# cyyever/distributed_learning_simulation_lib

Measured on AMD Instinct MI355X. Metric: aggregated GB/s (device-resident), N-client weighted FedAvg reduce, 1/2/4/8 GPU, higher is better.
Workload: dtype f64; 1 GPU; fedavg_resnet18_fp32_64_clients; clients_per_gpu=64, total_clients=64, clients_per_launch=64, client_table=prepared once (persistent client slots), params_per_client=11689512, tensors_per_client=62, in_dtype=float32, accumulate_dtype=float64, out_dtype=float32, parallelism=single GPU

## Files before the change

### distributed_learning_simulation_lib_amd/build.py

```python

from __future__ import annotations

import os
import shutil
import subprocess
from pathlib import Path

PKG_DIR = Path(__file__).resolve().parent
REPO_DIR = PKG_DIR.parent
CSRC = PKG_DIR / "csrc"
LIB_DIR = PKG_DIR / "_lib"
LIB_NAME = "libfedavg_hip.so"
LIB_PATH = LIB_DIR / LIB_NAME
SOURCES = [CSRC / "fedavg_kernels.hip", CSRC / "personalized_kernels.hip", CSRC / "robust_kernels.hip",
           CSRC / "krum_kernels.hip", CSRC / "point_kernels.hip", CSRC / "clip_kernels.hip", CSRC / "host_pack.cpp",
           CSRC / "sharded_comm.cpp", CSRC / "multi_device.cpp"]
HEADERS = [REPO_DIR / "include" / "fedavg_hip.h", CSRC / "exact_div.h", CSRC / "rccl_bind.h",
           CSRC / "robust_internal.h", CSRC / "krum_internal.h", CSRC / "point_internal.h", CSRC / "clip_internal.h"]
EXAMPLES = {"c_abi_round": REPO_DIR / "examples" / "c_abi_round.cpp",
            "multi_device_round": REPO_DIR / "examples" / "multi_device_round.cpp",
            "threaded_ranks": REPO_DIR / "tests" / "native" / "threaded_ranks.cpp"}
FAKE_RCCL_SRC = REPO_DIR / "tests" / "native" / "fake_rccl.cpp"
FAKE_RCCL = {"libfake_rccl.so": [], "libfake_rccl_nogather.so": ["-DFAKE_RCCL_NO_GATHER"]}
STAGING_SRC = CSRC / "staging_ext.cpp"
STAGING_NAME = "fedavg_staging"
STAGING_DIR = LIB_DIR / "staging"
STAGING_PATH = STAGING_DIR / f"{STAGING_NAME}.so"

HIPCC_FLAGS = [
    "--offload-arch=gfx950",
    "-O3",
    "-std=c++17",
    "-ffp-contract=off",
    "-fPIC",
    "-shared",
    "-Wall",
    "-Wno-unused-function",
]


def hipcc() -> str:
    cand = os.environ.get("HIPCC") or shutil.which("hipcc") or "/opt/rocm/bin/hipcc"
    return cand


def needs_build() -> bool:
    if not LIB_PATH.exists():
        return True
    mtime = LIB_PATH.stat().st_mtime
    return any(p.stat().st_mtime > mtime for p in SOURCES + HEADERS + [Path(__file__)])

# ... 74 lines not shown
```

### distributed_learning_simulation_lib_amd/csrc/fedavg_kernels.hip

```cpp
#include <hip/hip_runtime.h>
#include <hip/hip_ext.h>
#include <hip/hip_fp16.h>

#include <algorithm>
#include <atomic>
#include <chrono>
#include <cmath>
#include <cstdint>
#include <cstdio>
#include <cstdlib>
#include <cstring>
#include <limits>
#include <mutex>
#include <string>
#include <type_traits>
#include <vector>

#include "../../include/fedavg_hip.h"
#include "exact_div.h"
#include "robust_internal.h"
#include "krum_internal.h"
#include "point_internal.h"
#include "clip_internal.h"

namespace {

thread_local std::string g_last_error;

int32_t fail(int32_t code, const std::string& msg) {
  g_last_error = msg;
  return code;
}

#define FEDAVG_HIP_TRY(expr)                                                              \
  do {                                                                                    \
    hipError_t e_ = (expr);                                                               \
    if (e_ != hipSuccess) {                                                               \
      return fail(FEDAVG_ERR_HIP, std::string(#expr) + ": " + hipGetErrorString(e_));     \
    }                                                                                     \
  } while (0)

constexpr int kThreads = 256;
#ifndef FEDAVG_AE
#define FEDAVG_AE 16
#endif
#ifndef FEDAVG_AE_HALF
#define FEDAVG_AE_HALF 16
#endif
#ifndef FEDAVG_AE_F64
#define FEDAVG_AE_F64 8
#endif
#ifndef FEDAVG_TILE1
#define FEDAVG_TILE1 4096
#endif
#ifndef FEDAVG_CU_BYTES
#define FEDAVG_CU_BYTES 256
#endif
#ifndef FEDAVG_CU_BYTES_F64
#define FEDAVG_CU_BYTES_F64 512
#endif
#ifndef FEDAVG_PIPE
#define FEDAVG_PIPE 1
#endif
#ifndef FEDAVG_ACC_PLAIN_STORE_HALF
#define FEDAVG_ACC_PLAIN_STORE_HALF 1
#endif
#ifndef FEDAVG_BALANCE_DEFAULT
#define FEDAVG_BALANCE_DEFAULT 3
#endif
#ifndef FEDAVG_WALK_ALTERNATE
#define FEDAVG_WALK_ALTERNATE 1
#endif
#ifndef FEDAVG_PIPE_BYTES
#define FEDAVG_PIPE_BYTES 64
#endif
constexpr int kAE = FEDAVG_AE;
constexpr int kTile1 = FEDAVG_TILE1;
#ifndef FEDAVG_TILE_WIDE
#define FEDAVG_TILE_WIDE 8192
#endif
constexpr int kTileWide = FEDAVG_TILE_WIDE;
constexpr int kTile4 = (kThreads / 4) * kAE;

struct TileDesc {
  int32_t seg;
  int32_t count;
  int64_t start;
};

struct SegDesc {
  int64_t acc_off;
  int64_t numel;
};

struct CallTables {
  const void* const* cptrs;
  const double* w;
  const int32_t* kseg;
  const int32_t* acc_in;
  void* const* outs;
  const double* wtot;
  const void* const* base;
};

struct KArgs {
  const TileDesc* tiles;
  const SegDesc* segs;
  CallTables tab;
  double* acc;
  uint32_t* flag;
  int32_t tile_begin;
  int32_t num_tiles;
  int32_t K;
  int32_t zero_init;
  int32_t walk_back;
  const double* qtab;
  int32_t qtab_seg0;
  double* const* win_dst;
  const int32_t* win_edge;
  int32_t win_n;
  const double* const* comb_src;
// ... 108 lines not shown
  return (kptr<T>)(p);
}

__device__ __forceinline__ TileDesc load_tile(const TileDesc* tiles, int64_t i) {
  const kptr<int32_t> p = to_const<int32_t>(tiles + i);
  TileDesc d;
  d.seg = p[0];
  d.count = p[1];
  d.start = to_const<int64_t>(tiles + i)[1];
  return d;
}

template <typename T>
__device__ __forceinline__ double load_g(gptr<const T> p, int64_t i);
template <>
__device__ __forceinline__ double load_g<float>(gptr<const float> p, int64_t i) { return p[i]; }
template <>
__device__ __forceinline__ double load_g<double>(gptr<const double> p, int64_t i) { return p[i]; }
template <>
__device__ __forceinline__ double load_g<__half>(gptr<const __half> p, int64_t i) {
  return half_bits_to_f64(((gptr<const uint16_t>)p)[i]);
}
template <>
__device__ __forceinline__ double load_g<bf16_t>(gptr<const bf16_t> p, int64_t i) {
  return bf16_bits_to_f64(((gptr<const uint16_t>)p)[i]);
}

template <typename T, int LANES, bool FULL, bool VEC, int AE>
struct LaneLoader {
  using V = typename Vec16<T>::type;
  static constexpr int N = Vec16<T>::n;
  static constexpr int VPL = AE / N;

  __device__ __forceinline__ static void load_raw(gptr<const T> base, int li, V (&buf)[VPL], int nv = VPL) {
    const gptr<const V> vb = (gptr<const V>)base;
#pragma unroll
    for (int v = 0; v < VPL; ++v) {
      if (FULL || v < nv) {
        buf[v] = __builtin_nontemporal_load(vb + v * LANES + li);
      } else {
        buf[v] = V{};
      }
    }
  }

  __device__ __forceinline__ static void load_checked(gptr<const T> base, int li, int count,
                                                      double (&x)[AE]) {
#pragma unroll
    for (int v = 0; v < VPL; ++v) {
      const int e = (v * LANES + li) * N;
      if (VEC && e + N <= count) {
        const V raw = ((gptr<const V>)base)[v * LANES + li];
        expand<T>(raw, x + v * N);
      } else {
#pragma unroll
        for (int j = 0; j < N; ++j) x[v * N + j] = (e + j < count) ? load_g<T>(base, e + j) : 0.0;
      }
    }
  }
};

template <typename T, int SPLIT, int TILEN = kTile1>
struct Geo {
  static constexpr int AE = (SPLIT > 1) ? kAE
                          : (sizeof(T) == 2 ? FEDAVG_AE_HALF
                             : sizeof(T) == 8 ? FEDAVG_AE_F64
                                              : kAE);
  static constexpr int LANES = (SPLIT > 1) ? 64 : TILEN / AE;
  static constexpr int THREADS = (SPLIT > 1) ? kThreads : LANES;
  static constexpr int TILE = LANES * AE;
  static_assert(SPLIT == 1 || TILE == kTile4, "split tiles");
  static_assert(SPLIT > 1 || TILE == TILEN, "tile geometry");
  static_assert(THREADS % 64 == 0 && THREADS <= 1024, "workgroup size");
};

__device__ __forceinline__ void raise_flag(uint32_t* flag, int word) {
  __hip_atomic_store(flag + word, 1u, __ATOMIC_RELAXED, __HIP_MEMORY_SCOPE_SYSTEM);
}

template <typename V>
__device__ __forceinline__ void store_out(gptr<V> p, V v) {
  __builtin_nontemporal_store(v, p);
}

enum FoldKind : int { FOLD_MULADD = 0, FOLD_FMA = 1, FOLD_DELTA = 2 };

template <int FOLD>
__device__ __forceinline__ double fold(double acc, double x, double w, double base) {
  if constexpr (FOLD == FOLD_FMA) {
    return __builtin_fma(x, w, acc);
  } else if constexpr (FOLD == FOLD_DELTA) {
    const double full = base + x;
    const double p = full * w;
    return acc + p;
  } else {
    const double p = x * w;
    return acc + p;
  }
}

template <typename T, int OUT, int SPLIT, bool VEC, bool FULL, int FOLD, int TILEN = kTile1, bool PARTV = false,
          bool COMB = false>
__device__ __forceinline__ void tile_body(const KArgs& a, const TileDesc& td, double* lds) {
  constexpr int AE = Geo<T, SPLIT, TILEN>::AE;
  constexpr int LANES = Geo<T, SPLIT, TILEN>::LANES;
  using LL = LaneLoader<T, LANES, FULL && VEC, VEC, AE>;
  using V = typename LL::V;
  constexpr int N = LL::N;
  constexpr int VPL = LL::VPL;
  constexpr int CU_B = sizeof(T) == 8 ? FEDAVG_CU_BYTES_F64 : FEDAVG_CU_BYTES;
  constexpr int CU_LOADS = (CU_B / (VPL * 16)) < 2 ? 2 : (CU_B / (VPL * 16));
  constexpr bool FAST = (FULL || PARTV) && VEC;

  const int seg = td.seg;
  const int count = td.count;
  const int nv = FULL ? VPL : count / (LANES * N);
  const int wave = __builtin_amdgcn_readfirstlane(static_cast<int>(threadIdx.x) >> 6);
  const int li = (SPLIT == 1) ? static_cast<int>(threadIdx.x) : static_cast<int>(threadIdx.x & 63);

  const int kseg = to_const<int32_t>(a.tab.kseg)[seg];
  int kb = 0, ke = kseg;
  if constexpr (SPLIT > 1) {
    const int per = (kseg + SPLIT - 1) / SPLIT;
    kb = min(kseg, wave * per);
    ke = min(kseg, kb + per);
  }
  const kptr<uint64_t> cp = to_const<uint64_t>(a.tab.cptrs) + static_cast<int64_t>(seg) * a.K;
  const kptr<double> wp = to_const<double>(a.tab.w) + static_cast<int64_t>(seg) * a.K;
  const int64_t acc_base = to_const<int64_t>(a.segs)[2 * seg] + td.start;
  const int64_t elem_off = td.start * static_cast<int64_t>(sizeof(T));
  auto client = [&](int k) -> gptr<const T> {
    return to_global<T>(reinterpret_cast<const void*>(cp[k] + elem_off));
  };

  double acc[AE];
#pragma unroll
  for (int i = 0; i < AE; ++i) acc[i] = -0.0;
  bool have = a.zero_init != 0;
  if ((SPLIT == 1 || wave == 0) && !a.zero_init && to_const<int32_t>(a.tab.acc_in)[seg]) {
    const gptr<const double> ap = to_global<double>(a.acc + acc_base);
#pragma unroll
    for (int v = 0; v < VPL; ++v) {
      const int e = (v * LANES + li) * N;
#pragma unroll
      for (int j = 0; j < N; j += 2) {
        if (FULL || e + j + 2 <= count) {
          const f64x2 d = *(gptr<const f64x2>)(ap + e + j);
          acc[v * N + j] = d.x;
          acc[v * N + j + 1] = d.y;
        } else {
          if (e + j < count) acc[v * N + j] = ap[e + j];
          if (e + j + 1 < count) acc[v * N + j + 1] = ap[e + j + 1];
        }
      }
    }
    have = true;
  }

  double base[AE];
#pragma unroll
  for (int i = 0; i < AE; ++i) base[i] = 0.0;
  if constexpr (FOLD == FOLD_DELTA) {
    const gptr<const double> bp =
        to_global<double>(reinterpret_cast<const void*>(to_const<uint64_t>(a.tab.base)[seg])) + td.start;
#pragma unroll
    for (int v = 0; v < VPL; ++v) {
      const int e = (v * LANES + li) * N;
#pragma unroll
      for (int j = 0; j < N; j += 2) {
        if (VEC && (FULL || e + j + 2 <= count)) {
          const f64x2 d = *(gptr<const f64x2>)(bp + e + j);
          base[v * N + j] = d.x;
          base[v * N + j + 1] = d.y;
        } else {
          if (e + j < count) base[v * N + j] = bp[e + j];
          if (e + j + 1 < count) base[v * N + j + 1] = bp[e + j + 1];
        }
      }
    }
  }

  constexpr bool PIPE = FAST && ((FEDAVG_PIPE >> (sizeof(T) == 2 ? 0 : sizeof(T) == 4 ? 1 : 2)) & 1);
  if constexpr (PIPE) {
    constexpr int PB = FEDAVG_PIPE_BYTES;
    constexpr int PG = (PB / (VPL * 16)) < 1 ? 1 : (PB / (VPL * 16));
    V bufA[PG][VPL], bufB[PG][VPL];
    double wA[PG], wB[PG];
    auto load_stage = [&](V (&buf)[PG][VPL], double (&wk)[PG], int k) {
#pragma unroll
      for (int c = 0; c < PG; ++c) {
        const int kc = min(k + c, ke - 1);
        wk[c] = wp[kc];
        LL::load_raw(client(kc), li, buf[c], nv);
      }
    };
    auto fold_stage = [&](auto tail_tag, V (&buf)[PG][VPL], const double (&wk)[PG], int n) {
      constexpr bool TAIL = decltype(tail_tag)::value;
#pragma unroll
      for (int c = 0; c < PG; ++c) {
#pragma unroll
        for (int v = 0; v < VPL; ++v) {
          double x[N];
          expand<T>(buf[c][v], x);
#pragma unroll
          for (int j = 0; j < N; ++j) {
            double& r = acc[v * N + j];
            const double nv = fold<FOLD>(r, x[j], wk[c], base[v * N + j]);
            if constexpr (TAIL) {
              r = (c < n) ? nv : r;
            } else {
              r = nv;
            }
          }
        }
      }
    };
    if (kb < ke) {
      int k = kb;
      load_stage(bufA, wA, k);
      while (k + 2 * PG <= ke) {
        load_stage(bufB, wB, k + PG);
        fold_stage(std::false_type{}, bufA, wA, PG);
        load_stage(bufA, wA, k + 2 * PG);
        fold_stage(std::false_type{}, bufB, wB, PG);
        k += 2 * PG;
      }
      if (k + PG < ke) {
        load_stage(bufB, wB, k + PG);
        fold_stage(std::false_type{}, bufA, wA, PG);
        fold_stage(std::true_type{}, bufB, wB, ke - k - PG);
      } else if (k < ke) {
        fold_stage(std::true_type{}, bufA, wA, ke - k);
      }
    }
  } else if constexpr (FAST) {
    auto group = [&](auto tail_tag, int k, int n) {
      constexpr bool TAIL = decltype(tail_tag)::value;
      V buf[CU_LOADS][VPL];
      double wk[CU_LOADS];
#pragma unroll
      for (int c = 0; c < CU_LOADS; ++c) {
        const int kc = TAIL ? k + min(c, n - 1) : k + c;
        wk[c] = wp[kc];
        LL::load_raw(client(kc), li, buf[c], nv);
      }
#pragma unroll
      for (int c = 0; c < CU_LOADS; ++c) {
#pragma unroll
        for (int v = 0; v < VPL; ++v) {
          double x[N];
          expand<T>(buf[c][v], x);
#pragma unroll
          for (int j = 0; j < N; ++j) {
            double& r = acc[v * N + j];
            const double nv = fold<FOLD>(r, x[j], wk[c], base[v * N + j]);
            if constexpr (TAIL) {
              r = (c < n) ? nv : r;
            } else {
              r = nv;
            }
          }
        }
      }
    };
    int k = kb;
    for (; k + CU_LOADS <= ke; k += CU_LOADS) group(std::false_type{}, k, CU_LOADS);
    if (k < ke) group(std::true_type{}, k, ke - k);
  } else {
    for (int k = kb; k < ke; ++k) {
      const double wk = wp[k];
      double x[AE];
      LL::load_checked(client(k), li, count, x);
#pragma unroll
      for (int i = 0; i < AE; ++i) acc[i] = fold<FOLD>(acc[i], x[i], wk, base[i]);
    }
  }
  have = have || (ke > kb);

  if constexpr (SPLIT > 1) {
    int* have_lds = reinterpret_cast<int*>(lds + (SPLIT - 1) * 64 * AE);
    if (wave > 0) {
      double* dst = lds + ((wave - 1) * 64 + li) * AE;
#pragma unroll
      for (int i = 0; i < AE; ++i) dst[i] = acc[i];
      if (li == 0) have_lds[wave - 1] = have ? 1 : 0;
    }
    __syncthreads();
    if (wave != 0) return;
#pragma unroll
    for (int w2 = 1; w2 < SPLIT; ++w2) {
      if (have_lds[w2 - 1]) {
        const double* src = lds + ((w2 - 1) * 64 + li) * AE;
        if (have) {
#pragma unroll
          for (int i = 0; i < AE; ++i) acc[i] = acc[i] + src[i];
        } else {
#pragma unroll
          for (int i = 0; i < AE; ++i) acc[i] = src[i];
        }
        have = true;
      }
    }
  }
  if (!have) return;

  if constexpr (COMB) {
    static_assert(OUT != OUT_ACC && SPLIT == 1, "the own-window combine ends a final fold");
    double tot[AE];
#pragma unroll
    for (int i = 0; i < AE; ++i) tot[i] = -0.0;
    for (int h = 0; h < a.comb_n; ++h) {
      if (h == a.comb_self) {
#pragma unroll
        for (int i = 0; i < AE; ++i) tot[i] = tot[i] + acc[i];
      } else {
        const gptr<const double> sp =
            to_global<double>(reinterpret_cast<const void*>(to_const<uint64_t>(a.comb_src)[h])) + acc_base;
#pragma unroll
        for (int v = 0; v < VPL; ++v) {
          const int e = (v * LANES + li) * N;
#pragma unroll
          for (int j = 0; j < N; j += 2) {
            if (FULL || e + j + 2 <= count) {
              const f64x2 d = *(gptr<const f64x2>)(sp + e + j);
              tot[v * N + j] = tot[v * N + j] + d.x;
              tot[v * N + j + 1] = tot[v * N + j + 1] + d.y;
            } else {
              if (e + j < count) tot[v * N + j] = tot[v * N + j] + sp[e + j];
              if (e + j + 1 < count) tot[v * N + j + 1] = tot[v * N + j + 1] + sp[e + j + 1];
            }
          }
        }
      }
    }
#pragma unroll
    for (int i = 0; i < AE; ++i) acc[i] = tot[i];
  }

  bool bad_acc = false;
#pragma unroll
  for (int v = 0; v < VPL; ++v) {
    const int e = (v * LANES + li) * N;
#pragma unroll
    for (int j = 0; j < N; ++j) {
      const bool in_range = FULL || (e + j < count);
      bad_acc |= in_range && (acc[v * N + j] != acc[v * N + j]);
    }
  }

  if constexpr (OUT == OUT_ACC) {
    const gptr<double> ap = to_global_mut<double>(a.acc + acc_base);
#pragma unroll
    for (int v = 0; v < VPL; ++v) {
      const int e = (v * LANES + li) * N;
#pragma unroll
      for (int j = 0; j < N; j += 2) {
        if (FULL || e + j + 2 <= count) {
          const f64x2 pair = f64x2{acc[v * N + j], acc[v * N + j + 1]};
          if constexpr (sizeof(T) == 2 && FEDAVG_ACC_PLAIN_STORE_HALF) {
            *(gptr<f64x2>)(ap + e + j) = pair;
          } else {
            store_out((gptr<f64x2>)(ap + e + j), pair);
          }
        } else {
          if (e + j < count) ap[e + j] = acc[v * N + j];
          if (e + j + 1 < count) ap[e + j + 1] = acc[v * N + j + 1];
        }
      }
    }
    if (__ballot(bad_acc) != 0ull && (threadIdx.x & 63) == 0) raise_flag(a.flag, 0);
  } else {
    const double W = to_const<double>(a.tab.wtot)[seg];
    bool bad_res = false;
    double res[AE];
    exact_div_block<AE>(acc, res, W);
#pragma unroll
    for (int v = 0; v < VPL; ++v) {
      const int e = (v * LANES + li) * N;
#pragma unroll
      for (int j = 0; j < N; ++j) {
        const bool in_range = FULL || (e + j < count);
        bad_res |= in_range && (res[v * N + j] != res[v * N + j]);
      }
    }
    void* const out_raw = reinterpret_cast<void*>(to_const<uint64_t>(a.tab.outs)[seg]);
    if constexpr (OUT == OUT_F32) {
      const gptr<float> op = to_global_mut<float>(out_raw) + td.start;
#pragma unroll
      for (int v = 0; v < VPL; ++v) {
        const int e = (v * LANES + li) * N;
        if constexpr (N >= 4) {
#pragma unroll
          for (int j = 0; j < N; j += 4) {
            if (VEC && (FULL || e + j + 4 <= count)) {
              store_out((gptr<f32x4>)(op + e + j),
                  f32x4{static_cast<float>(res[v * N + j]), static_cast<float>(res[v * N + j + 1]),
                        static_cast<float>(res[v * N + j + 2]), static_cast<float>(res[v * N + j + 3])});
            } else {
#pragma unroll
              for (int q = 0; q < 4; ++q)
                if (e + j + q < count) op[e + j + q] = static_cast<float>(res[v * N + j + q]);
            }
          }
        } else {
          if (VEC && (FULL || e + 2 <= count)) {
            store_out((gptr<f32x2>)(op + e),
                      f32x2{static_cast<float>(res[v * N]), static_cast<float>(res[v * N + 1])});
          } else {
            if (e < count) op[e] = static_cast<float>(res[v * N]);
            if (e + 1 < count) op[e + 1] = static_cast<float>(res[v * N + 1]);
          }
        }
      }
    } else {
      const gptr<double> op = to_global_mut<double>(out_raw) + td.start;
#pragma unroll
      for (int v = 0; v < VPL; ++v) {
        const int e = (v * LANES + li) * N;
#pragma unroll
        for (int j = 0; j < N; j += 2) {
          if (VEC && (FULL || e + j + 2 <= count)) {
            store_out((gptr<f64x2>)(op + e + j), f64x2{res[v * N + j], res[v * N + j + 1]});
          } else {
            if (e + j < count) op[e + j] = res[v * N + j];
            if (e + j + 1 < count) op[e + j + 1] = res[v * N + j + 1];
          }
        }
      }
    }
    const uint64_t ba = __ballot(bad_acc);
    const uint64_t br = __ballot(bad_res);
    if ((ba | br) != 0ull && (threadIdx.x & 63) == 0) {
      if (ba) raise_flag(a.flag, 0);
      if (br) raise_flag(a.flag, 1);
    }
  }
}

template <typename T, int OUT, int SPLIT, bool VEC, int FOLD, int TILEN = kTile1, bool PV = false, bool COMB = false>
__global__ __launch_bounds__((Geo<T, SPLIT, TILEN>::THREADS)) void fedavg_tile_kernel(KArgs a) {
  __shared__ double lds[(SPLIT > 1) ? ((SPLIT - 1) * 64 * kAE + 8) : 1];
  constexpr int TILE = Geo<T, SPLIT, TILEN>::TILE;
  const int ntiles = (SPLIT == 1) ? a.num_tiles : static_cast<int>(gridDim.x);
  if constexpr (OUT == OUT_ACC && SPLIT == 1) {
    if (a.win_dst != nullptr) {
      for (int t = blockIdx.x; t < ntiles; t += gridDim.x) {
        const int32_t ti = a.tile_begin + t;
        const kptr<int32_t> we = to_const<int32_t>(a.win_edge);
        int j = 0;
        while (j + 1 < a.win_n && ti >= we[j + 1]) ++j;
        KArgs b = a;
        b.acc = reinterpret_cast<double*>(to_const<uint64_t>(a.win_dst)[j]);
        const TileDesc td = load_tile(a.tiles, ti);
        if (td.count == TILE) tile_body<T, OUT, SPLIT, VEC, true, FOLD, TILEN>(b, td, lds);
        else tile_body<T, OUT, SPLIT, VEC, false, FOLD, TILEN>(b, td, lds);
      }
      return;
    }
  }
  if constexpr (COMB) {
    const TileDesc td = load_tile(a.tiles, a.tile_begin + static_cast<int>(blockIdx.x));
    if (td.count == TILE) tile_body<T, OUT, SPLIT, VEC, true, FOLD, TILEN, false, true>(a, td, lds);
    else tile_body<T, OUT, SPLIT, VEC, false, FOLD, TILEN, false, true>(a, td, lds);
    return;
  }
  for (int t = blockIdx.x; t < ntiles; t += gridDim.x) {
    const TileDesc td = load_tile(a.tiles, a.tile_begin + (t < a.walk_back ? a.walk_back - 1 - t : t));
    constexpr int LV = Geo<T, SPLIT, TILEN>::LANES * Vec16<T>::n;
    if (td.count == TILE) {
      tile_body<T, OUT, SPLIT, VEC, true, FOLD, TILEN>(a, td, lds);
    } else {
      bool partv = false;
      if constexpr (PV && SPLIT == 1 && VEC && LV < TILE) partv = (td.count % LV) == 0;
      if (partv) {
        if constexpr (PV && SPLIT == 1 && VEC && LV < TILE) tile_body<T, OUT, SPLIT, VEC, false, FOLD, TILEN, true>(a, td, lds);
      } else {
        tile_body<T, OUT, SPLIT, VEC, false, FOLD, TILEN>(a, td, lds);
      }
    }
    if constexpr (SPLIT > 1) break;
  }
}

struct DynCtl {
  uint64_t word;
  uint64_t pad[7];
};
struct DynAck {
  uint64_t word;
  uint32_t error;
  uint32_t polls;
  uint64_t t_seen;
  uint64_t t_done;
  uint64_t t_rows;
};
struct DynMirror {
  uint64_t word;
  uint64_t pad[7];
};
constexpr int kDynCopies = 8;
constexpr int kDynMirrorSleep = 8;
constexpr int kDynTileSleep = 32;
__host__ __device__ constexpr uint64_t dyn_word(uint32_t count, uint32_t closed, uint32_t mode, uint32_t epoch) {
  return static_cast<uint64_t>(count & 0xffffffu) | (static_cast<uint64_t>(closed & 1u) << 24) |
         (static_cast<uint64_t>(mode & 7u) << 25) | (static_cast<uint64_t>(epoch) << 32);
}
struct DynArgs {
  const TileDesc* tiles;
  const TileDesc* edge_tiles;
  const SegDesc* segs;
  double* acc;
// ... 1155 lines not shown

namespace {

constexpr size_t align_up(size_t x, size_t a) { return (x + a - 1) / a * a; }

struct DynLayout {
  size_t ctl, ack, wtot, outs, wtab, ptab, bytes;
  DynLayout(int T, int cap) {
    ctl = 0;
    ack = align_up(ctl + sizeof(DynCtl), 64);
    wtot = align_up(ack + sizeof(DynAck), 64);
    outs = align_up(wtot + sizeof(double) * T, 64);
    wtab = align_up(outs + sizeof(uint64_t) * T, 64);
    ptab = align_up(wtab + sizeof(double) * cap, 64);
    bytes = align_up(ptab + sizeof(uint64_t) * static_cast<size_t>(T) * cap, 4096);
  }
};


int32_t elem_size(int32_t dt) {
  switch (dt) {
    case FEDAVG_F32: return 4;
    case FEDAVG_F16: return 2;
    case FEDAVG_BF16: return 2;
    case FEDAVG_F64: return 8;
    case FEDAVG_QSGD_F32: return 1;
    case FEDAVG_QSGD_F64: return 1;
    case FEDAVG_NNADQ_F32: return 1;
    case FEDAVG_NNADQ_F64: return 1;
    default: return 0;
  }
}

int32_t build_balanced_tiles(const std::vector<int64_t>& numel, int tile, int gran, int64_t slots,
                             std::vector<TileDesc>& out) {
  std::vector<TileDesc> full, tail;
  int64_t tail_elems = 0;
  for (size_t t = 0; t < numel.size(); ++t) {
    const int64_t q = numel[t] / tile;
    for (int64_t i = 0; i < q; ++i) full.push_back(TileDesc{static_cast<int32_t>(t), tile, i * tile});
    int64_t start = q * tile, r = numel[t] - q * tile;
    const int64_t rv = r - r % gran;
    if (rv > 0) {
      tail.push_back(TileDesc{static_cast<int32_t>(t), static_cast<int32_t>(rv), start});
      start += rv;
      r -= rv;
      tail_elems += rv;
    }
    if (r > 0) {
      tail.push_back(TileDesc{static_cast<int32_t>(t), static_cast<int32_t>(r), start});
      tail_elems += r;
    }
  }
  slots = std::max<int64_t>(slots, 1);
  const int64_t head = (static_cast<int64_t>(full.size()) / slots) * slots;
  const int64_t rest = static_cast<int64_t>(full.size()) - head;
  const int64_t remaining = rest * tile + tail_elems;
  int64_t piece = (remaining + slots - 1) / slots;
  piece = std::min<int64_t>(tile, std::max<int64_t>(gran, (piece + gran - 1) / gran * gran));
  out.assign(full.begin(), full.begin() + head);
  std::vector<TileDesc> end;
  for (int64_t i = head; i < static_cast<int64_t>(full.size()); ++i) {
    for (int64_t s = 0; s < tile; s += piece) {
      const int64_t c = std::min<int64_t>(piece, tile - s);
      end.push_back(TileDesc{full[i].seg, static_cast<int32_t>(c), full[i].start + s});
    }
  }
  end.insert(end.end(), tail.begin(), tail.end());
  std::stable_sort(end.begin(), end.end(), [](const TileDesc& a, const TileDesc& b) { return a.count > b.count; });
  out.insert(out.end(), end.begin(), end.end());
  return static_cast<int32_t>(head);
}

void build_tiles(const std::vector<int64_t>& numel, int tile, std::vector<TileDesc>& out) {
  out.clear();
  for (size_t t = 0; t < numel.size(); ++t) {
    for (int64_t s = 0; s < numel[t]; s += tile) {
      TileDesc d;
      d.seg = static_cast<int32_t>(t);
      d.count = static_cast<int32_t>(std::min<int64_t>(tile, numel[t] - s));
      d.start = s;
      out.push_back(d);
    }
  }
}

bool stream_idle(hipStream_t s) { return hipStreamQuery(s) == hipSuccess || hipStreamQuery(s) == hipSuccess; }

hipEvent_t take_event(fedavg_ctx* c) {
  if (!c->event_pool.empty()) {
    hipEvent_t e = c->event_pool.back();
    c->event_pool.pop_back();
    return e;
  }
  hipEvent_t e = nullptr;
  if (hipEventCreate(&e) != hipSuccess) return nullptr;
  return e;
}

struct Staged {
  CallTables tab;
  int32_t Kmax = 0;
  int32_t stride = 1;
  bool aligned = true;
  bool clients_aligned = true;
  bool delta = false;
  int32_t max_weight_bits = 0;
  bool weights_tame = true;
  double last_weight = std::numeric_limits<double>::quiet_NaN();
  std::vector<int32_t> kseg;
};

}

struct fedavg_plan {
  enum Kind { AGGREGATE = 0, PARTIAL = 1, FINALIZE = 2 };
  fedavg_ctx* ctx = nullptr;
// ... 506 lines not shown
}

int out_kind_of(int32_t out_dtype) {
  if (out_dtype == FEDAVG_F32) return OUT_F32;
  if (out_dtype == FEDAVG_F64) return OUT_F64;
  return -1;
}

#define FEDAVG_RET(expr)            \
  do {                              \
    int32_t r_ = (expr);            \
    if (r_ != FEDAVG_OK) return r_; \
  } while (0)

}

extern "C" __attribute__((visibility("hidden"))) int32_t fedavg_internal_pers_constant(const char* name, int64_t* out);

extern "C" {

int32_t fedavg_abi_version(void) { return FEDAVG_ABI_VERSION; }

int32_t fedavg_build_flags(void) {
  return 0;
}

int32_t fedavg_kernel_constant(const char* name, int64_t* out) {
  if (name == nullptr || out == nullptr) return fail(FEDAVG_ERR_INVALID, "null argument");
  const std::string n(name);
  int64_t v = -1;
  if (n == "tile") v = kTile1;
  else if (n == "tile_wide") v = kTileWide;
  else if (n == "split_tile") v = kTile4;
  else if (n == "qsgd_tile") v = kTile1;
  else if (n == "qsgd_ae") v = kQsgdAE;
  else if (n == "qsgd_group") v = kQsgdGroup;
  else if (n == "nnadq_tile") v = kTile1;
  else if (n == "nnadq_ae") v = kNnadqAE;
  else if (n == "nnadq_group") v = kNnadqGroup;
  else if (n == "nnadq_header") v = kNnadqHeader;
  else if (n.rfind("pers_", 0) == 0) {
    if (fedavg_internal_pers_constant(name, &v) != FEDAVG_OK) v = -1;
  } else if (n.rfind("robust_", 0) == 0 || n.rfind("mam_", 0) == 0) {
    if (fedavg_internal_robust_constant(name, &v) != FEDAVG_OK) v = -1;
  } else if (n.rfind("krum_", 0) == 0) {
    if (fedavg_internal_krum_constant(name, &v) != FEDAVG_OK) v = -1;
  } else if (n.rfind("point_", 0) == 0) {
    if (fedavg_internal_point_constant(name, &v) != FEDAVG_OK) v = -1;
  } else if (n.rfind("clip_", 0) == 0) {
    if (fedavg_internal_clip_constant(name, &v) != FEDAVG_OK) v = -1;
  } else {
    const auto dsep = n.rfind('_');
    const std::string key = dsep == std::string::npos ? n : n.substr(0, dsep);
    const std::string d = dsep == std::string::npos ? "" : n.substr(dsep + 1);
    auto pick = [&](auto tag) {
      using T = decltype(tag);
      using GW = Geo<T, 1, (sizeof(T) < 8 && kTileWide > 0) ? kTileWide : kTile1>;
      using G1 = Geo<T, 1, kTile1>;
      constexpr int VPLW = GW::AE / Vec16<T>::n;
      constexpr int CU_B = sizeof(T) == 8 ? FEDAVG_CU_BYTES_F64 : FEDAVG_CU_BYTES;
      constexpr int GROUP = (CU_B / (VPLW * 16)) < 2 ? 2 : (CU_B / (VPLW * 16));
      constexpr bool PIPE = (FEDAVG_PIPE >> (sizeof(T) == 2 ? 0 : sizeof(T) == 4 ? 1 : 2)) & 1;
      constexpr int PG = (FEDAVG_PIPE_BYTES / (VPLW * 16)) < 1 ? 1 : (FEDAVG_PIPE_BYTES / (VPLW * 16));
      if (key == "ae") v = GW::AE;
      else if (key == "lanes") v = GW::LANES;
      else if (key == "ae4096") v = G1::AE;
// ... 37 lines not shown
    if (seg_numel[t] <= 0) return fail(FEDAVG_ERR_INVALID, "segment with no elements");
    if (seg_numel[t] > (int64_t(1) << 40)) return fail(FEDAVG_ERR_INVALID, "segment too large");
  }
  if (reinterpret_cast<uintptr_t>(accumulator) % 16 != 0)
    return fail(FEDAVG_ERR_INVALID, "accumulator must be 16-byte aligned");
  FEDAVG_HIP_TRY(hipSetDevice(device));
  fedavg_ctx* c = new fedavg_ctx();
  c->device = device;
  c->T = num_segments;
  c->seg_numel.assign(seg_numel, seg_numel + num_segments);
  c->seg_acc_off.resize(num_segments);
  int64_t off = 0;
  for (int t = 0; t < num_segments; ++t) {
    c->seg_acc_off[t] = off;
    off += static_cast<int64_t>(align_up(static_cast<size_t>(seg_numel[t]), FEDAVG_ACC_ALIGN));
  }
  c->acc_numel = off;
  c->wsum.assign(num_segments, -0.0);
  if (const char* e = std::getenv("FEDAVG_WIDE_MIN_CLIENTS")) c->wide_min_clients = std::atoi(e);
  if (const char* e = std::getenv("FEDAVG_WALK_ALTERNATE")) c->walk_alternate = std::atoi(e) != 0;
  if (const char* e = std::getenv("FEDAVG_QSGD_TABLE_CAP")) {
    const long long v = std::atoll(e);
    if (v > 0) c->qtab_cap_bytes = static_cast<size_t>(v);
  }
  c->valid.assign(num_segments, 0);
  build_tiles(c->seg_numel, kTile1, c->tiles1);
  build_tiles(c->seg_numel, kTile4, c->tiles4);
  if (kTileWide > 0) build_tiles(c->seg_numel, kTileWide, c->tilesw);
  {
    const char* env = std::getenv("FEDAVG_BALANCE");
    const int bal = env ? std::atoi(env) : FEDAVG_BALANCE_DEFAULT;
    const char* always_env = std::getenv("FEDAVG_BALANCE_ALWAYS");
    const bool always = always_env && std::atoi(always_env) != 0;
    int cus = 0;
    if (bal && hipDeviceGetAttribute(&cus, hipDeviceAttributeMultiprocessorCount, device) == hipSuccess && cus > 0) {
      int per_cu = 0;
      auto thin_tail = [&](size_t tiles, int64_t slots) {
        const int64_t rem = static_cast<int64_t>(tiles) % slots;
        return always || (tiles > static_cast<size_t>(slots) && rem > 0 && 2 * rem < slots);
      };
      if ((bal & 1) && kTileWide > 0 &&
          hipOccupancyMaxActiveBlocksPerMultiprocessor(
              &per_cu, reinterpret_cast<const void*>(&fedavg_tile_kernel<float, OUT_F32, 1, true, FOLD_FMA, kTileWide, true>),
              Geo<float, 1, kTileWide>::THREADS, 0) == hipSuccess && per_cu > 0 &&
          thin_tail(c->tilesw.size(), static_cast<int64_t>(per_cu) * cus))
        c->tilesw_bal_head =
            build_balanced_tiles(c->seg_numel, kTileWide, Geo<float, 1, kTileWide>::LANES * Vec16<float>::n,
                                 static_cast<int64_t>(per_cu) * cus, c->tilesw_bal);
      per_cu = 0;
      if ((bal & 2) &&
          hipOccupancyMaxActiveBlocksPerMultiprocessor(
              &per_cu, reinterpret_cast<const void*>(&fedavg_tile_kernel<double, OUT_F32, 1, true, FOLD_FMA, kTile1, true>),
              Geo<double, 1, kTile1>::THREADS, 0) == hipSuccess && per_cu > 0 &&
          thin_tail(c->tiles1.size(), static_cast<int64_t>(per_cu) * cus))
        c->tiles1_bal_head =
            build_balanced_tiles(c->seg_numel, kTile1, Geo<double, 1, kTile1>::LANES * Vec16<double>::n,
                                 static_cast<int64_t>(per_cu) * cus, c->tiles1_bal);
    }
  }
  if (c->tiles1.size() > static_cast<size_t>(INT32_MAX / 2)) {
    delete c;
    return fail(FEDAVG_ERR_INVALID, "layout too large");
  }
  std::vector<SegDesc> segs(num_segments);
  for (int t = 0; t < num_segments; ++t) segs[t] = SegDesc{c->seg_acc_off[t], c->seg_numel[t]};

  auto cleanup = [&](hipError_t e, const char* what) {
    fedavg_ctx_destroy(c);
    return fail(FEDAVG_ERR_HIP, std::string(what) + ": " + hipGetErrorString(e));
  };
  hipError_t e;
  if ((e = hipMalloc(reinterpret_cast<void**>(&c->d_tiles1), sizeof(TileDesc) * c->tiles1.size())) != hipSuccess)
    return cleanup(e, "hipMalloc tiles1");
  if ((e = hipMalloc(reinterpret_cast<void**>(&c->d_tiles4), sizeof(TileDesc) * c->tiles4.size())) != hipSuccess)
    return cleanup(e, "hipMalloc tiles4");
  if ((e = hipMalloc(reinterpret_cast<void**>(&c->d_segs), sizeof(SegDesc) * segs.size())) != hipSuccess)
    return cleanup(e, "hipMalloc segs");
  if ((e = hipHostMalloc(reinterpret_cast<void**>(&c->h_flag), sizeof(uint32_t) * 4,
                         hipHostMallocMapped | hipHostMallocCoherent)) != hipSuccess)
    return cleanup(e, "hipHostMalloc flag");
  if ((e = hipHostGetDevicePointer(reinterpret_cast<void**>(&c->d_flag), c->h_flag, 0)) != hipSuccess)
    return cleanup(e, "hipHostGetDevicePointer flag");
  if ((e = hipMemcpy(c->d_tiles1, c->tiles1.data(), sizeof(TileDesc) * c->tiles1.size(), hipMemcpyHostToDevice)) != hipSuccess)
    return cleanup(e, "hipMemcpy tiles1");
  if ((e = hipMemcpy(c->d_tiles4, c->tiles4.data(), sizeof(TileDesc) * c->tiles4.size(), hipMemcpyHostToDevice)) != hipSuccess)
    return cleanup(e, "hipMemcpy tiles4");
  if (!c->tilesw.empty()) {
    if ((e = hipMalloc(reinterpret_cast<void**>(&c->d_tilesw), sizeof(TileDesc) * c->tilesw.size())) != hipSuccess)
      return cleanup(e, "hipMalloc tilesw");
    if ((e = hipMemcpy(c->d_tilesw, c->tilesw.data(), sizeof(TileDesc) * c->tilesw.size(), hipMemcpyHostToDevice)) !=
// ... 1426 lines not shown
```

Before: 6387 GB/s.

## Model-driven tail tile balancing with exact-length pieces and short-tile kernel path

Replaces the fixed-piece tail balancer with a search over piece lengths that keeps per-segment runs contiguous, cuts them into row-aligned pieces and picks the cut minimising a simulated greedy makespan across block slots. The kernel gains compile-time specialisations for pieces of 1–3 rows, so loads lose the per-vector bound checks, and a dedicated path for sub-row tails that gathers 16 clients per group. The aim is to shrink the end-of-grid tail and the divergent masked work on partial tiles, at the cost of more template instantiations and a heuristic cost model.

```diff
diff --git a/distributed_learning_simulation_lib_amd/build.py b/distributed_learning_simulation_lib_amd/build.py
--- a/distributed_learning_simulation_lib_amd/build.py
+++ b/distributed_learning_simulation_lib_amd/build.py
@@ -16,7 +16,8 @@
            CSRC / "krum_kernels.hip", CSRC / "point_kernels.hip", CSRC / "clip_kernels.hip", CSRC / "host_pack.cpp",
            CSRC / "sharded_comm.cpp", CSRC / "multi_device.cpp"]
 HEADERS = [REPO_DIR / "include" / "fedavg_hip.h", CSRC / "exact_div.h", CSRC / "rccl_bind.h",
-           CSRC / "robust_internal.h", CSRC / "krum_internal.h", CSRC / "point_internal.h", CSRC / "clip_internal.h"]
+           CSRC / "robust_internal.h", CSRC / "krum_internal.h", CSRC / "point_internal.h", CSRC / "clip_internal.h",
+           CSRC / "tile_order.h"]
 EXAMPLES = {"c_abi_round": REPO_DIR / "examples" / "c_abi_round.cpp",
             "multi_device_round": REPO_DIR / "examples" / "multi_device_round.cpp",
             "threaded_ranks": REPO_DIR / "tests" / "native" / "threaded_ranks.cpp"}
diff --git a/distributed_learning_simulation_lib_amd/csrc/fedavg_kernels.hip b/distributed_learning_simulation_lib_amd/csrc/fedavg_kernels.hip
--- a/distributed_learning_simulation_lib_amd/csrc/fedavg_kernels.hip
+++ b/distributed_learning_simulation_lib_amd/csrc/fedavg_kernels.hip
@@ -22,6 +22,8 @@
 #include "krum_internal.h"
 #include "point_internal.h"
 #include "clip_internal.h"
+
+#include "tile_order.h"
 
 namespace {
 
@@ -68,6 +70,9 @@
 #ifndef FEDAVG_BALANCE_DEFAULT
 #define FEDAVG_BALANCE_DEFAULT 3
 #endif
+#ifndef FEDAVG_SHORT_GROUP
+#define FEDAVG_SHORT_GROUP 16
+#endif
 #ifndef FEDAVG_WALK_ALTERNATE
 #define FEDAVG_WALK_ALTERNATE 1
 #endif
@@ -82,11 +87,6 @@
 constexpr int kTileWide = FEDAVG_TILE_WIDE;
 constexpr int kTile4 = (kThreads / 4) * kAE;
 
-struct TileDesc {
-  int32_t seg;
-  int32_t count;
-  int64_t start;
-};
 
 struct SegDesc {
   int64_t acc_off;
@@ -261,16 +261,10 @@
   static constexpr int N = Vec16<T>::n;
   static constexpr int VPL = AE / N;
 
-  __device__ __forceinline__ static void load_raw(gptr<const T> base, int li, V (&buf)[VPL], int nv = VPL) {
+  __device__ __forceinline__ static void load_raw(gptr<const T> base, int li, V (&buf)[VPL]) {
     const gptr<const V> vb = (gptr<const V>)base;
 #pragma unroll
-    for (int v = 0; v < VPL; ++v) {
-      if (FULL || v < nv) {
-        buf[v] = __builtin_nontemporal_load(vb + v * LANES + li);
-      } else {
-        buf[v] = V{};
-      }
-    }
+    for (int v = 0; v < VPL; ++v) buf[v] = __builtin_nontemporal_load(vb + v * LANES + li);
   }
 
   __device__ __forceinline__ static void load_checked(gptr<const T> base, int li, int count,
@@ -328,24 +322,32 @@
   }
 }
 
-template <typename T, int OUT, int SPLIT, bool VEC, bool FULL, int FOLD, int TILEN = kTile1, bool PARTV = false,
-          bool COMB = false>
+template <typename T, int OUT, int SPLIT, bool VEC, bool FULL, int FOLD, int TILEN = kTile1, int NV = 0,
+          bool COMB = false, bool SHORT = false>
 __device__ __forceinline__ void tile_body(const KArgs& a, const TileDesc& td, double* lds) {
-  constexpr int AE = Geo<T, SPLIT, TILEN>::AE;
+  constexpr bool PARTV = NV > 0;
+  static_assert(!(PARTV && (FULL || SHORT)) && !(FULL && SHORT), "one kind of tile");
+  static_assert(!SHORT || (SPLIT == 1 && sizeof(T) >= 4), "the short path: exact order, 4- / 8-byte inputs");
+  constexpr int N = Vec16<T>::n;
+  constexpr int AE = PARTV ? NV * N : SHORT ? N : Geo<T, SPLIT, TILEN>::AE;
+  static_assert(AE <= Geo<T, SPLIT, TILEN>::AE, "a piece is shorter than its tile");
   constexpr int LANES = Geo<T, SPLIT, TILEN>::LANES;
-  using LL = LaneLoader<T, LANES, FULL && VEC, VEC, AE>;
+  constexpr bool WHOLE = FULL || PARTV;
+  using LL = LaneLoader<T, LANES, WHOLE && VEC, VEC, AE>;
   using V = typename LL::V;
-  constexpr int N = LL::N;
   constexpr int VPL = LL::VPL;
   constexpr int CU_B = sizeof(T) == 8 ? FEDAVG_CU_BYTES_F64 : FEDAVG_CU_BYTES;
-  constexpr int CU_LOADS = (CU_B / (VPL * 16)) < 2 ? 2 : (CU_B / (VPL * 16));
-  constexpr bool FAST = (FULL || PARTV) && VEC;
+  constexpr int CU_RAW = (CU_B / (VPL * 16)) < 2 ? 2 : (CU_B / (VPL * 16));
+  constexpr int CU_LOADS = (PARTV && CU_RAW > 8) ? 8 : CU_RAW;
+  constexpr bool FAST = WHOLE && VEC;
 
   const int seg = td.seg;
   const int count = td.count;
-  const int nv = FULL ? VPL : count / (LANES * N);
   const int wave = __builtin_amdgcn_readfirstlane(static_cast<int>(threadIdx.x) >> 6);
   const int li = (SPLIT == 1) ? static_cast<int>(threadIdx.x) : static_cast<int>(threadIdx.x & 63);
+  if constexpr (SHORT) {
+    if (wave * 64 * N >= count) return;
+  }
 
   const int kseg = to_const<int32_t>(a.tab.kseg)[seg];
   int kb = 0, ke = kseg;
@@ -373,7 +375,7 @@
       const int e = (v * LANES + li) * N;
 #pragma unroll
       for (int j = 0; j < N; j += 2) {
-        if (FULL || e + j + 2 <= count) {
+        if (WHOLE || e + j + 2 <= count) {
           const f64x2 d = *(gptr<const f64x2>)(ap + e + j);
           acc[v * N + j] = d.x;
           acc[v * N + j + 1] = d.y;
@@ -397,7 +399,7 @@
       const int e = (v * LANES + li) * N;
 #pragma unroll
       for (int j = 0; j < N; j += 2) {
-        if (VEC && (FULL || e + j + 2 <= count)) {
+        if (VEC && (WHOLE || e + j + 2 <= count)) {
           const f64x2 d = *(gptr<const f64x2>)(bp + e + j);
           base[v * N + j] = d.x;
           base[v * N + j + 1] = d.y;
@@ -420,7 +422,7 @@
       for (int c = 0; c < PG; ++c) {
         const int kc = min(k + c, ke - 1);
         wk[c] = wp[kc];
-        LL::load_raw(client(kc), li, buf[c], nv);
+        LL::load_raw(client(kc), li, buf[c]);
       }
     };
     auto fold_stage = [&](auto tail_tag, V (&buf)[PG][VPL], const double (&wk)[PG], int n) {
@@ -471,7 +473,7 @@
       for (int c = 0; c < CU_LOADS; ++c) {
         const int kc = TAIL ? k + min(c, n - 1) : k + c;
         wk[c] = wp[kc];
-        LL::load_raw(client(kc), li, buf[c], nv);
+        LL::load_raw(client(kc), li, buf[c]);
       }
 #pragma unroll
       for (int c = 0; c < CU_LOADS; ++c) {
@@ -495,6 +497,37 @@
     int k = kb;
     for (; k + CU_LOADS <= ke; k += CU_LOADS) group(std::false_type{}, k, CU_LOADS);
     if (k < ke) group(std::true_type{}, k, ke - k);
+  } else if constexpr (SHORT) {
+    constexpr int SG = FEDAVG_SHORT_GROUP;
+    int idx[N];
+#pragma unroll
+    for (int j = 0; j < N; ++j) idx[j] = min(li * N + j, count - 1);
+    auto group = [&](auto tail_tag, int k, int n) {
+      constexpr bool TAIL = decltype(tail_tag)::value;
+      T raw[SG][N];
+#pragma unroll
+      for (int c = 0; c < SG; ++c) {
+        const gptr<const T> p = client(TAIL ? k + min(c, n - 1) : k + c);
+#pragma unroll
+        for (int j = 0; j < N; ++j) raw[c][j] = p[idx[j]];
+      }
+#pragma unroll
+      for (int c = 0; c < SG; ++c) {
+        const double wk = wp[TAIL ? k + min(c, n - 1) : k + c];
+#pragma unroll
+        for (int j = 0; j < N; ++j) {
+          const double nx = fold<FOLD>(acc[j], to_f64(raw[c][j]), wk, base[j]);
+          if constexpr (TAIL) {
+            acc[j] = (c < n) ? nx : acc[j];
+          } else {
+            acc[j] = nx;
+          }
+        }
+      }
+    };
+    int k = kb;
+    for (; k + SG <= ke; k += SG) group(std::false_type{}, k, SG);
+    if (k < ke) group(std::true_type{}, k, ke - k);
   } else {
     for (int k = kb; k < ke; ++k) {
       const double wk = wp[k];
@@ -550,7 +583,7 @@
           const int e = (v * LANES + li) * N;
 #pragma unroll
           for (int j = 0; j < N; j += 2) {
-            if (FULL || e + j + 2 <= count) {
+            if (WHOLE || e + j + 2 <= count) {
               const f64x2 d = *(gptr<const f64x2>)(sp + e + j);
               tot[v * N + j] = tot[v * N + j] + d.x;
               tot[v * N + j + 1] = tot[v * N + j + 1] + d.y;
@@ -572,7 +605,7 @@
     const int e = (v * LANES + li) * N;
 #pragma unroll
     for (int j = 0; j < N; ++j) {
-      const bool in_range = FULL || (e + j < count);
+      const bool in_range = WHOLE || (e + j < count);
       bad_acc |= in_range && (acc[v * N + j] != acc[v * N + j]);
     }
   }
@@ -584,7 +617,7 @@
       const int e = (v * LANES + li) * N;
 #pragma unroll
       for (int j = 0; j < N; j += 2) {
-        if (FULL || e + j + 2 <= count) {
+        if (WHOLE || e + j + 2 <= count) {
           const f64x2 pair = f64x2{acc[v * N + j], acc[v * N + j + 1]};
           if constexpr (sizeof(T) == 2 && FEDAVG_ACC_PLAIN_STORE_HALF) {
             *(gptr<f64x2>)(ap + e + j) = pair;
@@ -608,7 +641,7 @@
       const int e = (v * LANES + li) * N;
 #pragma unroll
       for (int j = 0; j < N; ++j) {
-        const bool in_range = FULL || (e + j < count);
+        const bool in_range = WHOLE || (e + j < count);
         bad_res |= in_range && (res[v * N + j] != res[v * N + j]);
       }
     }
@@ -621,7 +654,7 @@
         if constexpr (N >= 4) {
 #pragma unroll
           for (int j = 0; j < N; j += 4) {
-            if (VEC && (FULL || e + j + 4 <= count)) {
+            if (VEC && (WHOLE || e + j + 4 <= count)) {
               store_out((gptr<f32x4>)(op + e + j),
                   f32x4{static_cast<float>(res[v * N + j]), static_cast<float>(res[v * N + j + 1]),
                         static_cast<float>(res[v * N + j + 2]), static_cast<float>(res[v * N + j + 3])});
@@ -632,7 +665,7 @@
             }
           }
         } else {
-          if (VEC && (FULL || e + 2 <= count)) {
+          if (VEC && (WHOLE || e + 2 <= count)) {
             store_out((gptr<f32x2>)(op + e),
                       f32x2{static_cast<float>(res[v * N]), static_cast<float>(res[v * N + 1])});
           } else {
@@ -648,7 +681,7 @@
         const int e = (v * LANES + li) * N;
 #pragma unroll
         for (int j = 0; j < N; j += 2) {
-          if (VEC && (FULL || e + j + 2 <= count)) {
+          if (VEC && (WHOLE || e + j + 2 <= count)) {
             store_out((gptr<f64x2>)(op + e + j), f64x2{res[v * N + j], res[v * N + j + 1]});
           } else {
             if (e + j < count) op[e + j] = res[v * N + j];
@@ -689,23 +722,32 @@
   }
   if constexpr (COMB) {
     const TileDesc td = load_tile(a.tiles, a.tile_begin + static_cast<int>(blockIdx.x));
-    if (td.count == TILE) tile_body<T, OUT, SPLIT, VEC, true, FOLD, TILEN, false, true>(a, td, lds);
-    else tile_body<T, OUT, SPLIT, VEC, false, FOLD, TILEN, false, true>(a, td, lds);
+    static_assert(!PV, "the own-window combine runs the plain order");
+    if (td.count == TILE) tile_body<T, OUT, SPLIT, VEC, true, FOLD, TILEN, 0, true>(a, td, lds);
+    else tile_body<T, OUT, SPLIT, VEC, false, FOLD, TILEN, 0, true>(a, td, lds);
     return;
   }
   for (int t = blockIdx.x; t < ntiles; t += gridDim.x) {
     const TileDesc td = load_tile(a.tiles, a.tile_begin + (t < a.walk_back ? a.walk_back - 1 - t : t));
     constexpr int LV = Geo<T, SPLIT, TILEN>::LANES * Vec16<T>::n;
+    constexpr int ROWS = TILE / LV;
+    constexpr bool PIECES = PV && SPLIT == 1 && VEC && ROWS > 1;
+    constexpr bool SHORTS = PV && SPLIT == 1 && VEC && sizeof(T) == 4 && FEDAVG_SHORT_GROUP > 0;
+    static_assert(!PIECES || ROWS <= 4, "one case per piece length below");
     if (td.count == TILE) {
       tile_body<T, OUT, SPLIT, VEC, true, FOLD, TILEN>(a, td, lds);
+    } else if (PIECES && td.count % LV == 0) {
+      if constexpr (PIECES) {
+        switch (td.count / LV) {
+          case 1: tile_body<T, OUT, SPLIT, VEC, false, FOLD, TILEN, 1>(a, td, lds); break;
+          case 2: if constexpr (ROWS > 2) tile_body<T, OUT, SPLIT, VEC, false, FOLD, TILEN, 2>(a, td, lds); break;
+          default: if constexpr (ROWS > 3) tile_body<T, OUT, SPLIT, VEC, false, FOLD, TILEN, 3>(a, td, lds); break;
+        }
+      }
+    } else if (SHORTS && td.count < LV) {
+      if constexpr (SHORTS) tile_body<T, OUT, SPLIT, VEC, false, FOLD, TILEN, 0, false, true>(a, td, lds);
     } else {
-      bool partv = false;
-      if constexpr (PV && SPLIT == 1 && VEC && LV < TILE) partv = (td.count % LV) == 0;
-      if (partv) {
-        if constexpr (PV && SPLIT == 1 && VEC && LV < TILE) tile_body<T, OUT, SPLIT, VEC, false, FOLD, TILEN, true>(a, td, lds);
-      } else {
-        tile_body<T, OUT, SPLIT, VEC, false, FOLD, TILEN>(a, td, lds);
-      }
+      tile_body<T, OUT, SPLIT, VEC, false, FOLD, TILEN>(a, td, lds);
     }
     if constexpr (SPLIT > 1) break;
   }
@@ -1927,57 +1969,21 @@
   }
 }
 
-int32_t build_balanced_tiles(const std::vector<int64_t>& numel, int tile, int gran, int64_t slots,
-                             std::vector<TileDesc>& out) {
-  std::vector<TileDesc> full, tail;
-  int64_t tail_elems = 0;
-  for (size_t t = 0; t < numel.size(); ++t) {
-    const int64_t q = numel[t] / tile;
-    for (int64_t i = 0; i < q; ++i) full.push_back(TileDesc{static_cast<int32_t>(t), tile, i * tile});
-    int64_t start = q * tile, r = numel[t] - q * tile;
-    const int64_t rv = r - r % gran;
-    if (rv > 0) {
-      tail.push_back(TileDesc{static_cast<int32_t>(t), static_cast<int32_t>(rv), start});
-      start += rv;
-      r -= rv;
-      tail_elems += rv;
-    }
-    if (r > 0) {
-      tail.push_back(TileDesc{static_cast<int32_t>(t), static_cast<int32_t>(r), start});
-      tail_elems += r;
-    }
-  }
-  slots = std::max<int64_t>(slots, 1);
-  const int64_t head = (static_cast<int64_t>(full.size()) / slots) * slots;
-  const int64_t rest = static_cast<int64_t>(full.size()) - head;
-  const int64_t remaining = rest * tile + tail_elems;
-  int64_t piece = (remaining + slots - 1) / slots;
-  piece = std::min<int64_t>(tile, std::max<int64_t>(gran, (piece + gran - 1) / gran * gran));
-  out.assign(full.begin(), full.begin() + head);
-  std::vector<TileDesc> end;
-  for (int64_t i = head; i < static_cast<int64_t>(full.size()); ++i) {
-    for (int64_t s = 0; s < tile; s += piece) {
-      const int64_t c = std::min<int64_t>(piece, tile - s);
-      end.push_back(TileDesc{full[i].seg, static_cast<int32_t>(c), full[i].start + s});
-    }
-  }
-  end.insert(end.end(), tail.begin(), tail.end());
-  std::stable_sort(end.begin(), end.end(), [](const TileDesc& a, const TileDesc& b) { return a.count > b.count; });
-  out.insert(out.end(), end.begin(), end.end());
-  return static_cast<int32_t>(head);
-}
-
-void build_tiles(const std::vector<int64_t>& numel, int tile, std::vector<TileDesc>& out) {
-  out.clear();
-  for (size_t t = 0; t < numel.size(); ++t) {
-    for (int64_t s = 0; s < numel[t]; s += tile) {
-      TileDesc d;
-      d.seg = static_cast<int32_t>(t);
-      d.count = static_cast<int32_t>(std::min<int64_t>(tile, numel[t] - s));
-      d.start = s;
-      out.push_back(d);
-    }
-  }
+int64_t whole_layout_slots(int32_t dtype, int device) {
+  int cus = 0, per_cu = 0;
+  if (hipDeviceGetAttribute(&cus, hipDeviceAttributeMultiprocessorCount, device) != hipSuccess || cus <= 0) return 0;
+  hipError_t e = hipErrorInvalidValue;
+  if (dtype == FEDAVG_F32 && kTileWide > 0) {
+    e = hipOccupancyMaxActiveBlocksPerMultiprocessor(
+        &per_cu, reinterpret_cast<const void*>(&fedavg_tile_kernel<float, OUT_F32, 1, true, FOLD_FMA, kTileWide, true>),
+        Geo<float, 1, kTileWide>::THREADS, 0);
+  } else if (dtype == FEDAVG_F64) {
+    e = hipOccupancyMaxActiveBlocksPerMultiprocessor(
+        &per_cu, reinterpret_cast<const void*>(&fedavg_tile_kernel<double, OUT_F32, 1, true, FOLD_FMA, kTile1, true>),
+        Geo<double, 1, kTile1>::THREADS, 0);
+  }
+  if (e != hipSuccess || per_cu <= 0) return 0;
+  return static_cast<int64_t>(per_cu) * cus;
 }
 
 bool stream_idle(hipStream_t s) { return hipStreamQuery(s) == hipSuccess || hipStreamQuery(s) == hipSuccess; }
@@ -2550,6 +2556,12 @@
   if (n == "tile") v = kTile1;
   else if (n == "tile_wide") v = kTileWide;
   else if (n == "split_tile") v = kTile4;
+  else if (n == "short_group_f32") v = FEDAVG_SHORT_GROUP;
+  else if (n == "slots_f32" || n == "slots_f64") {
+    int dev = 0;
+    if (hipGetDevice(&dev) == hipSuccess) v = whole_layout_slots(n == "slots_f32" ? FEDAVG_F32 : FEDAVG_F64, dev);
+    if (v <= 0) v = -1;
+  }
   else if (n == "qsgd_tile") v = kTile1;
   else if (n == "qsgd_ae") v = kQsgdAE;
   else if (n == "qsgd_group") v = kQsgdGroup;
@@ -2653,30 +2665,19 @@
     const int bal = env ? std::atoi(env) : FEDAVG_BALANCE_DEFAULT;
     const char* always_env = std::getenv("FEDAVG_BALANCE_ALWAYS");
     const bool always = always_env && std::atoi(always_env) != 0;
-    int cus = 0;
-    if (bal && hipDeviceGetAttribute(&cus, hipDeviceAttributeMultiprocessorCount, device) == hipSuccess && cus > 0) {
-      int per_cu = 0;
-      auto thin_tail = [&](size_t tiles, int64_t slots) {
+    if (bal) {
+      auto partial_tail = [&](size_t tiles, int64_t slots, bool thin_only) {
         const int64_t rem = static_cast<int64_t>(tiles) % slots;
-        return always || (tiles > static_cast<size_t>(slots) && rem > 0 && 2 * rem < slots);
+        return always || (tiles > static_cast<size_t>(slots) && rem > 0 && (!thin_only || 2 * rem < slots));
       };
-      if ((bal & 1) && kTileWide > 0 &&
-          hipOccupancyMaxActiveBlocksPerMultiprocessor(
-              &per_cu, reinterpret_cast<const void*>(&fedavg_tile_kernel<float, OUT_F32, 1, true, FOLD_FMA, kTileWide, true>),
-              Geo<float, 1, kTileWide>::THREADS, 0) == hipSuccess && per_cu > 0 &&
-          thin_tail(c->tilesw.size(), static_cast<int64_t>(per_cu) * cus))
-        c->tilesw_bal_head =
-            build_balanced_tiles(c->seg_numel, kTileWide, Geo<float, 1, kTileWide>::LANES * Vec16<float>::n,
-                                 static_cast<int64_t>(per_cu) * cus, c->tilesw_bal);
-      per_cu = 0;
-      if ((bal & 2) &&
-          hipOccupancyMaxActiveBlocksPerMultiprocessor(
-              &per_cu, reinterpret_cast<const void*>(&fedavg_tile_kernel<double, OUT_F32, 1, true, FOLD_FMA, kTile1, true>),
-              Geo<double, 1, kTile1>::THREADS, 0) == hipSuccess && per_cu > 0 &&
-          thin_tail(c->tiles1.size(), static_cast<int64_t>(per_cu) * cus))
-        c->tiles1_bal_head =
-            build_balanced_tiles(c->seg_numel, kTile1, Geo<double, 1, kTile1>::LANES * Vec16<double>::n,
-                                 static_cast<int64_t>(per_cu) * cus, c->tiles1_bal);
+      const int64_t slots32 = whole_layout_slots(FEDAVG_F32, device);
+      if ((bal & 1) && kTileWide > 0 && slots32 > 0 && partial_tail(c->tilesw.size(), slots32, true))
+        c->tilesw_bal_head = build_balanced_tiles(
+            c->seg_numel, kTileWide, Geo<float, 1, kTileWide>::LANES * Vec16<float>::n, slots32, c->tilesw_bal);
+      const int64_t slots64 = whole_layout_slots(FEDAVG_F64, device);
+      if ((bal & 2) && slots64 > 0 && partial_tail(c->tiles1.size(), slots64, true))
+        c->tiles1_bal_head = build_balanced_tiles(
+            c->seg_numel, kTile1, Geo<double, 1, kTile1>::LANES * Vec16<double>::n, slots64, c->tiles1_bal);
     }
   }
   if (c->tiles1.size() > static_cast<size_t>(INT32_MAX / 2)) {
diff --git a/distributed_learning_simulation_lib_amd/csrc/tile_order.h b/distributed_learning_simulation_lib_amd/csrc/tile_order.h
--- /dev/null
+++ b/distributed_learning_simulation_lib_amd/csrc/tile_order.h
@@ -0,0 +1,111 @@
+#pragma once
+
+#include <algorithm>
+#include <cstdint>
+#include <functional>
+#include <queue>
+#include <vector>
+
+struct TileDesc {
+  int32_t seg;
+  int32_t count;
+  int64_t start;
+};
+
+inline void build_tiles(const std::vector<int64_t>& numel, int tile, std::vector<TileDesc>& out) {
+  out.clear();
+  for (size_t t = 0; t < numel.size(); ++t) {
+    for (int64_t s = 0; s < numel[t]; s += tile) {
+      TileDesc d;
+      d.seg = static_cast<int32_t>(t);
+      d.count = static_cast<int32_t>(std::min<int64_t>(tile, numel[t] - s));
+      d.start = s;
+      out.push_back(d);
+    }
+  }
+}
+
+struct TileEndModel {
+  double fixed = 1.4;
+  double row = 1.0;
+  double short_tile = 1.8;
+  double cost(int64_t count, int gran) const {
+    if (count < gran) return short_tile;
+    return fixed + row * static_cast<double>((count + gran - 1) / gran);
+  }
+};
+
+inline double tile_end_makespan(const std::vector<double>& costs, int64_t slots) {
+  std::priority_queue<double, std::vector<double>, std::greater<double>> free_at;
+  double end = 0.0;
+  for (double c : costs) {
+    double t0 = 0.0;
+    if (static_cast<int64_t>(free_at.size()) >= slots) {
+      t0 = free_at.top();
+      free_at.pop();
+    }
+    free_at.push(t0 + c);
+    end = std::max(end, t0 + c);
+  }
+  return end;
+}
+
+inline int32_t build_balanced_tiles(const std::vector<int64_t>& numel, int tile, int gran, int64_t slots,
+                                    std::vector<TileDesc>& out, const TileEndModel& model = TileEndModel()) {
+  slots = std::max<int64_t>(slots, 1);
+  const int64_t rows_per_tile = tile / gran;
+  int64_t nfull = 0;
+  for (int64_t n : numel) nfull += n / tile;
+  const int64_t head = (nfull / slots) * slots;
+  out.clear();
+  out.reserve(static_cast<size_t>(nfull) + 2 * numel.size());
+  struct Run {
+    int32_t seg;
+    int64_t start, rows;
+  };
+  std::vector<Run> runs;
+  std::vector<TileDesc> ragged;
+  int64_t seen = 0;
+  for (size_t t = 0; t < numel.size(); ++t) {
+    const int64_t q = numel[t] / tile;
+    const int64_t in_head = std::min<int64_t>(q, std::max<int64_t>(0, head - seen));
+    for (int64_t i = 0; i < in_head; ++i) out.push_back(TileDesc{static_cast<int32_t>(t), tile, i * tile});
+    seen += q;
+    const int64_t start = in_head * tile;
+    const int64_t rows = (numel[t] - start) / gran;
+    if (rows > 0) runs.push_back(Run{static_cast<int32_t>(t), start, rows});
+    const int64_t r = numel[t] - start - rows * gran;
+    if (r > 0) ragged.push_back(TileDesc{static_cast<int32_t>(t), static_cast<int32_t>(r), start + rows * gran});
+  }
+  auto cut = [&](int64_t R, std::vector<TileDesc>& end) {
+    end.clear();
+    for (const Run& run : runs) {
+      const int64_t pieces = (run.rows + R - 1) / R;
+      const int64_t lo = run.rows / pieces, extra = run.rows % pieces;
+      int64_t s = run.start;
+      for (int64_t p = 0; p < pieces; ++p) {
+        const int64_t c = (lo + (p < extra ? 1 : 0)) * gran;
+        end.push_back(TileDesc{run.seg, static_cast<int32_t>(c), s});
+        s += c;
+      }
+    }
+    end.insert(end.end(), ragged.begin(), ragged.end());
+    std::stable_sort(end.begin(), end.end(), [&](const TileDesc& a, const TileDesc& b) {
+      return model.cost(a.count, gran) > model.cost(b.count, gran);
+    });
+  };
+  std::vector<TileDesc> end, best;
+  double best_span = -1.0;
+  for (int64_t R = rows_per_tile; R >= 1; --R) {
+    cut(R, end);
+    std::vector<double> costs(end.size());
+    for (size_t i = 0; i < end.size(); ++i) costs[i] = model.cost(end[i].count, gran);
+    const double span = tile_end_makespan(costs, slots);
+    if (best_span < 0.0 || span < best_span) {
+      best_span = span;
+      best.swap(end);
+    }
+  }
+  out.insert(out.end(), best.begin(), best.end());
+  return static_cast<int32_t>(head);
+}
```

New measurement: 6378 GB/s. Within noise of the previous version (-0.1%).
